# zkHubHQ/distributed-groth16

Measured on AMD Instinct MI355X. Metric: groth16_constraints_per_sec, higher is better.
Workload: dtype u32; 1 GPU; BN254 Groth16 prove from the matrices, synthetic R1CS with 2^20 - 2 constraints (3 nonzeros per row of A and B), 2^20 wires, 2 instance variables; r, s != 0 (R1CS x witness + 6 NTTs of 2^20 + 4 G1 MSMs + 1 G2 MSM); proving key RESIDENT as window tables (built once per key outside the timed region); curve=bn254, log_domain=20, parallelism=single GPU, key_table_bytes=6039807360, key_table_stride=1

## Files before the change

distributed-groth16_amd/csrc/msm_geom.h:

```cpp
#pragma once
#include <stddef.h>
#include <stdint.h>
#include <stdlib.h>

#ifndef DG_HD
#if defined(__HIPCC__)
#define DG_HD __host__ __device__ __forceinline__
#else
#define DG_HD inline
#endif
#endif

namespace dg16 {

constexpr unsigned kMinSegLog = 3, kMaxSegLog = 9;
constexpr unsigned kMinLanesLog = 18;
constexpr unsigned kGiantSegs = 64;
constexpr unsigned kGiantSlices = 64;
constexpr unsigned kGiantSliceSegs = 512;

struct MsmGeom {
  unsigned c;
  unsigned nwin;
  unsigned log_nb;
  unsigned seg_log;
  unsigned seg_cap;
  unsigned bw;
  unsigned table;
  unsigned rows;
  size_t region;
};

inline unsigned msm_window_bits(size_t n, bool table, unsigned scalar_bits = 0) {
  unsigned lg = 0;
  while (((size_t)1 << (lg + 1)) <= n) lg++;
  if (n > ((size_t)3 << lg) / 2) lg++;
  int c = table ? (int)lg - 3 : (int)lg - 4;
  if (table && c < 16) {
    c = (int)lg + 1 < 16 ? (int)lg + 1 : 16;
    if (scalar_bits && lg >= 13) {
      auto top = [&](int w) { const int bits = (int)scalar_bits + 1; return bits - ((bits + w - 1) / w - 1) * w; };
      const int t15 = top(15), t16 = top(16);
      if (t15 >= t16) c = (t15 > t16 || lg <= 16) ? 15 : 16;
    }
  }
  if (const char* e = getenv(table ? "DG16_MSM_TABLE_C" : "DG16_MSM_C")) c = atoi(e);
  int hi = table ? 20 : 16;
  if (c < 4) c = 4;
  if (c > hi) c = hi;
  return (unsigned)c;
}

inline MsmGeom msm_geometry(size_t n, unsigned scalar_bits, bool table = false, unsigned c_fixed = 0, unsigned stride = 1) {
  MsmGeom g;
  g.c = c_fixed ? c_fixed : msm_window_bits(n, table, table ? scalar_bits : 0);
  g.nwin = (scalar_bits + 1 + g.c - 1) / g.c;
  g.log_nb = g.c - 1;
  g.table = table ? 1u : 0u;
  if (stride < 1) stride = 1;
  if (stride > g.nwin) stride = g.nwin;
  g.bw = table ? stride : g.nwin;
  g.rows = (g.nwin + g.bw - 1) / g.bw;
  g.region = (size_t)g.rows * n;
  {
    size_t mean = g.region >> g.log_nb;
    unsigned lm = 0;
    while (((size_t)2 << lm) <= mean) lm++;
    unsigned le_all = 0;
    while (((size_t)2 << le_all) <= g.region * g.bw) le_all++;
    int sl = (int)le_all - 20;
    if (sl < 4) sl = 4;
    if (sl > 5) sl = 5;
    if (sl > (int)lm - 2) sl = (int)lm - 2;
    if (sl < 4) sl = 4;
    unsigned le = 0;
    while (((size_t)2 << le) <= (size_t)g.nwin * n) le++;
    int cap = (int)le - (int)kMinLanesLog;
    if (!table && le == 20 && cap < 4) cap = 4;
    if (sl > cap) sl = cap;
    g.seg_log = (unsigned)(sl < (int)kMinSegLog ? (int)kMinSegLog : sl > (int)kMaxSegLog ? (int)kMaxSegLog : sl);
    static const int seg_env = [] { const char* e = getenv("DG16_MSM_SEG_LOG"); return e ? atoi(e) : 0; }();
    if (seg_env >= (int)kMinSegLog && seg_env <= (int)kMaxSegLog) g.seg_log = (unsigned)seg_env;
  }
  g.seg_cap = (1u << g.log_nb) + (unsigned)((g.region + (1u << g.seg_log) - 1) >> g.seg_log);
  return g;
}

constexpr unsigned kScanBlock = 4096;

constexpr unsigned kPartScalars = 1024;
constexpr unsigned kPartMax = 256;
constexpr unsigned kPartMaxLowBits = 12;
constexpr unsigned kPartTileLog = 11;
constexpr unsigned kPartBlocks = 32;

struct PartGeom {
  unsigned low_bits, nparts, nblk1;
};
struct PartPlan {
  PartGeom pg;
  bool partitioned;
};
inline PartPlan msm_partition_plan(const MsmGeom& g, size_t n) {
  const size_t nbw = (size_t)g.bw << g.log_nb;
  unsigned lg_nbw = 0;
  while (((size_t)1 << lg_nbw) < nbw) lg_nbw++;
  static const int force_path = [] { const char* e = getenv("DG16_MSM_SORT"); return e ? atoi(e) : 0; }();
  PartPlan p;
  p.pg.low_bits = lg_nbw > 8 ? lg_nbw - 8 : 0;
  p.partitioned = p.pg.low_bits <= kPartMaxLowBits &&
                  (force_path == 2 || (force_path != 1 && (size_t)g.nwin * n >= ((size_t)1 << 18)));
  p.pg.nparts = (unsigned)((nbw + ((size_t)1 << p.pg.low_bits) - 1) >> p.pg.low_bits);
  p.pg.nblk1 = (unsigned)((n + kPartScalars - 1) / kPartScalars);
  return p;
}

constexpr unsigned kRowLog = 8;
struct RowGeom {
  unsigned row_log;
  unsigned rows_log;
};
inline RowGeom row_geometry(const MsmGeom& g) {
  RowGeom r;
  r.row_log = g.log_nb < kRowLog ? g.log_nb : kRowLog;
  r.rows_log = g.log_nb - r.row_log;
  return r;
}
constexpr size_t kLaneReduceMaxBuckets = 32768;

DG_HD void giant_geometry(unsigned nseg, unsigned& slices, unsigned& per) {
  slices = (nseg + kGiantSliceSegs - 1) / kGiantSliceSegs;
  if (slices > kGiantSlices) slices = kGiantSlices;
  per = (nseg + slices - 1) / slices;
  slices = (nseg + per - 1) / per;
}

constexpr int kGlvBits = 127;
constexpr int kGlv4Bits = 65;

struct PlainPlan {
  bool split;
  unsigned c_small;
  unsigned scalar_bits;
};
inline PlainPlan msm_plain_plan(bool nine_limbs, unsigned dim, size_t n, bool split_applies) {
  PlainPlan p{false, 0u, 0u};
  if (!split_applies || !n || !((size_t)dim * n * 40 < ((size_t)1 << 31))) return p;
  p.split = true;
  p.scalar_bits = dim == 2 ? (unsigned)kGlvBits : (unsigned)kGlv4Bits;
  if (dim == 2) {
    const unsigned c0 = msm_window_bits(2 * n, false);
    if (nine_limbs && (c0 == 7 || c0 == 9) && !getenv("DG16_MSM_C")) p.c_small = 8;
    if ((c0 == 14 || c0 == 15) && !getenv("DG16_MSM_C")) p.c_small = 16;
  }
  return p;
}

constexpr unsigned kMaxTableWin = 64;
inline unsigned table_stride_for(size_t full_bytes, size_t budget, unsigned nwin) {
  if (!budget || full_bytes <= budget || nwin <= 1) return 1;
  const size_t row = full_bytes / nwin;
  size_t rows_fit = budget / (row ? row : 1);
  if (rows_fit < 1) rows_fit = 1;
  unsigned k = (unsigned)((nwin + rows_fit - 1) / rows_fit);
  return k < 1 ? 1 : k > nwin ? nwin : k;
}

}
```

distributed-groth16_amd/csrc/msm_reduce_impl.h:

```cpp
#pragma once
#include "msm_impl.h"

#ifndef DG16_REDUCE_PRIO
#define DG16_REDUCE_PRIO 0
#endif
namespace dg16 {


template <class T>
__device__ __forceinline__ T lane_xor_words(const T& v, int mask) {
  static_assert(sizeof(T) % 4 == 0, "word-sized type");
  T r;
  const uint32_t* src = reinterpret_cast<const uint32_t*>(&v);
  uint32_t* dst = reinterpret_cast<uint32_t*>(&r);
#pragma unroll
  for (unsigned i = 0; i < sizeof(T) / 4; i++) dst[i] = (uint32_t)__shfl_xor((int)src[i], mask);
  return r;
}

template <class F>
__global__ void __launch_bounds__(256) msm_giant_kernel(MsmGeom g, unsigned wg_log, const unsigned* __restrict__ counts,
                                                         const unsigned* __restrict__ seg_off,
                                                         XYZZ29<F>* __restrict__ seg_sum,
                                                         const unsigned* __restrict__ giant_count,
                                                         const unsigned* __restrict__ giant_list, unsigned giant_cap) {
  __builtin_amdgcn_s_setprio(DG16_REDUCE_PRIO);
  __shared__ XYZZ29<F> sh[256];
  unsigned nwork = giant_count[1];
  if (nwork > 2 * giant_cap) nwork = 2 * giant_cap;
  const unsigned* work = giant_list + giant_cap;
  for (unsigned wi = blockIdx.x; wi < nwork; wi += gridDim.x) {
    const unsigned item = work[wi];
    const unsigned gid = giant_list[DG_IDX(11, item >> 6, giant_cap)], slice = item & 63;
    const unsigned wy = gid >> g.log_nb;
    const size_t gs = ((size_t)(wy % g.bw) << g.log_nb) + (gid & ((1u << g.log_nb) - 1));
    const unsigned k = (counts[gs] + (1u << g.seg_log) - 1) >> g.seg_log, first = seg_off[gs];
    const unsigned nseg = msm_nparts(first, k, wg_log);
    unsigned slices, per;
    giant_geometry(nseg, slices, per);
    XYZZ29<F>* sp = seg_sum + (size_t)wy * g.seg_cap;
    const unsigned lo = slice * per;
    const unsigned hi = lo + per < nseg ? lo + per : nseg;
    sh[threadIdx.x] = XYZZ29<F>::inf();
    __syncthreads();
    const unsigned iters = (hi - lo + 255) >> 8;
#pragma unroll 1
    for (unsigned step = 0; step < iters + 8; step++) {
      const XYZZ29<F>* b;
      bool on;
      if (step < iters) {
        const unsigned s = lo + step * 256 + threadIdx.x;
        on = s < hi;
        b = &sp[DG_IDX(12, msm_part_slot(first, on ? s : lo, wg_log), g.seg_cap)];
      } else {
        const unsigned stride = 128u >> (step - iters);
        on = threadIdx.x < stride;
        b = &sh[(threadIdx.x + stride) & 255];
      }
      if (on) XYZZ29<F>::add_mem(&sh[threadIdx.x], &sh[threadIdx.x], b);
      __syncthreads();
    }
    if (threadIdx.x == 0) sp[DG_IDX(12, msm_part_slot(first, lo, wg_log), g.seg_cap)] = sh[0];
    __syncthreads();
  }
}

template <class F>
__global__ void __launch_bounds__(64) msm_giant_fold_kernel(MsmGeom g, unsigned wg_log, const unsigned* __restrict__ counts,
                                                             const unsigned* __restrict__ seg_off,
                                                             const XYZZ29<F>* __restrict__ seg_sum,
                                                             XYZZ29<F>* __restrict__ buckets,
                                                             const unsigned* __restrict__ giant_count,
                                                             const unsigned* __restrict__ giant_list,
                                                             unsigned giant_cap) {
  __builtin_amdgcn_s_setprio(DG16_REDUCE_PRIO);
  __shared__ XYZZ29<F> sh[kGiantSlices];
  unsigned ng = *giant_count;
  if (ng > giant_cap) ng = giant_cap;
  for (unsigned gi = blockIdx.x; gi < ng; gi += gridDim.x) {
    const unsigned gid = giant_list[gi];
    const unsigned wy = gid >> g.log_nb;
    const size_t gs = ((size_t)(wy % g.bw) << g.log_nb) + (gid & ((1u << g.log_nb) - 1));
    const unsigned k = (counts[gs] + (1u << g.seg_log) - 1) >> g.seg_log, first = seg_off[gs];
    const unsigned nseg = msm_nparts(first, k, wg_log);
    unsigned slices, per;
    giant_geometry(nseg, slices, per);
    const XYZZ29<F>* sp = seg_sum + (size_t)wy * g.seg_cap;
    sh[threadIdx.x] = threadIdx.x < slices ? sp[DG_IDX(12, msm_part_slot(first, threadIdx.x * per, wg_log), g.seg_cap)] : XYZZ29<F>::inf();
    __syncthreads();
#pragma unroll 1
    for (unsigned stride = kGiantSlices / 2; stride > 0; stride >>= 1) {
      if (threadIdx.x < stride) XYZZ29<F>::add_mem(&sh[threadIdx.x], &sh[threadIdx.x], &sh[threadIdx.x + stride]);
      __syncthreads();
    }
    if (threadIdx.x == 0) buckets[gid] = sh[0];
    __syncthreads();
  }
}


constexpr unsigned kCoopTreeMax = 64;
template <class F>
__device__ __forceinline__ void tree_step_coop(XYZZ29<F>* sh, unsigned base, unsigned d) {
  const unsigned row16 = (threadIdx.x >> 4) & 15u;
#pragma unroll 1
  for (unsigned i = row16; i < d; i += 16) {
    const XYZZ29<F> v = add_wave29(sh[base + i], sh[base + i + d]);
    if ((threadIdx.x & 15u) == 0) sh[base + i] = v;
  }
}

template <class F>
__global__ void __launch_bounds__(256) msm_row_kernel(MsmGeom g, RowGeom rg, const XYZZ29<F>* __restrict__ buckets,
                                                       XYZZ29<F>* __restrict__ row_w, XYZZ29<F>* __restrict__ row_r) {
  __builtin_amdgcn_s_setprio(DG16_REDUCE_PRIO);
  __shared__ XYZZ29<F> sh[256];
  const unsigned c = threadIdx.x, row = 1u << rg.row_log;
  const size_t rid = ((size_t)blockIdx.y << rg.rows_log) + blockIdx.x;
  sh[c] = c < row ? buckets[(rid << rg.row_log) + c] : XYZZ29<F>::inf();
  __syncthreads();
#pragma unroll 1
  for (unsigned step = 0; step < 2 * rg.row_log; step++) {
    const bool scan = step < rg.row_log;
    const unsigned d = scan ? 1u << step : row >> (step - rg.row_log + 1);
    const bool on = scan ? c + d < row : c < d;
    if (step == rg.row_log && c == 0) row_r[rid] = sh[0];
    if (!scan && d <= kCoopTreeMax) {
      __syncthreads();
      tree_step_coop<F>(sh, 0u, d);
      __syncthreads();
      continue;
    }
    XYZZ29<F> v;
    if (on) XYZZ29<F>::add_mem(&v, &sh[c], &sh[(c + d) & 255]);
    __syncthreads();
    if (on) sh[c] = v;
    __syncthreads();
  }
  if (c == 0) {
    if (rg.row_log == 0) row_r[rid] = sh[0];
    row_w[rid] = sh[0];
  }
}

template <class F, int LANES>
__global__ void __launch_bounds__(LANES) msm_rowchunk_kernel(unsigned log_nb, unsigned k_log,
                                                              const XYZZ29<F>* __restrict__ buckets,
                                                              XYZZ29<F>* __restrict__ fold ) {
  __builtin_amdgcn_s_setprio(DG16_REDUCE_PRIO);
  constexpr unsigned LL = LANES == 256 ? 8u : 7u;
  static_assert(LANES == 256 || LANES == 128, "workgroup of 256 or 128 lanes");
  __shared__ XYZZ29<F> s_r[LANES];
  __shared__ XYZZ29<F> s_w[LANES];
  const unsigned j = threadIdx.x, K = 1u << k_log;
  const XYZZ29<F>* B = buckets + ((size_t)blockIdx.y << log_nb) + (((size_t)blockIdx.x * LANES + j) << k_log);
  XYZZ29<F>* out = fold + (size_t)blockIdx.y * 3 * 256;
  s_r[j] = XYZZ29<F>::inf();
  s_w[j] = XYZZ29<F>::inf();
  __syncthreads();
  const unsigned s_scan = 2 * K, s_tree = s_scan + LL, n_steps = s_tree + LL;
#pragma unroll 1
  for (unsigned step = 0; step < n_steps; step++) {
    const XYZZ29<F>*a, *b;
    XYZZ29<F>* dst;
    bool on = true;
    if (step < s_scan) {
      const bool even = (step & 1) == 0;
      dst = even ? &s_r[j] : &s_w[j];
      a = dst;
      b = even ? &B[K - 1 - (step >> 1)] : &s_r[j];
    } else if (step < s_tree) {
      const unsigned d = 1u << (step - s_scan);
      on = j + d < (unsigned)LANES;
      dst = &s_r[j];
      a = dst;
      b = &s_r[(j + d) & (LANES - 1)];
    } else {
      if (step == s_tree) {
        if (j == 0) {
          out[1 * 256 + blockIdx.x] = s_r[0];
          s_r[0] = XYZZ29<F>::inf();
        }
        __syncthreads();
      }
      const unsigned d = (unsigned)LANES >> (step - s_tree + 1);
      const unsigned c = j & (LANES / 2 - 1);
      XYZZ29<F>* arr = j < LANES / 2 ? s_r : s_w;
      on = c < d;
      dst = &arr[c];
      a = dst;
      b = &arr[(c + d) & (LANES - 1)];
    }
    XYZZ29<F> v;
    if (on) XYZZ29<F>::add_mem(&v, a, b);
    __syncthreads();
    if (on) *dst = v;
    __syncthreads();
  }
  if (j == 0) out[2 * 256 + blockIdx.x] = s_r[0];
  if (j == LANES / 2) out[0 * 256 + blockIdx.x] = s_w[0];
}

template <class F>
__global__ void __launch_bounds__(64) msm_rowfold_kernel(RowGeom rg, const XYZZ29<F>* __restrict__ row_w,
                                                          const XYZZ29<F>* __restrict__ row_r,
                                                          XYZZ29<F>* __restrict__ fold ) {
  __builtin_amdgcn_s_setprio(DG16_REDUCE_PRIO);
  __shared__ XYZZ29<F> st[64][2];
  const unsigned gid = blockIdx.x * 64 + threadIdx.x;
  const unsigned half = gid >> 8, t = gid & 255;
  const unsigned per_log = rg.rows_log - 8, per = 1u << per_log;
  const size_t base = ((size_t)blockIdx.y << rg.rows_log) + (size_t)t * per;
  XYZZ29<F>* run = &st[threadIdx.x][0];
  XYZZ29<F>* acc = &st[threadIdx.x][1];
  *run = XYZZ29<F>::inf();
  *acc = XYZZ29<F>::inf();
#pragma unroll 1
  for (unsigned k = 0; k < 2 * per; k++) {
    const unsigned j = per - 1 - (k >> 1);
    const bool first = (k & 1) == 0;
    const bool on = first ? (half == 1 && j + 1 < per) : true;
    const XYZZ29<F>* b = first ? run : (half == 0 ? row_w : row_r) + base + j;
    if (on) XYZZ29<F>::add_mem(first ? acc : run, first ? acc : run, b);
  }
  XYZZ29<F>* out = fold + (size_t)blockIdx.y * 3 * 256;
  out[half * 256 + t] = *run;
  if (half == 1) out[2 * 256 + t] = *acc;
}

struct TopGeom {
  unsigned folded, per_log, lanes, final_log, rows_log;
};
template <class F, int HALVES>
__global__ void __launch_bounds__(256 * HALVES) msm_top_kernel(TopGeom tg, const XYZZ29<F>* __restrict__ row_w,
                                                                const XYZZ29<F>* __restrict__ row_r,
                                                                const XYZZ29<F>* __restrict__ fold,
                                                                XYZZ29<F>* __restrict__ window_sums) {
  __builtin_amdgcn_s_setprio(DG16_REDUCE_PRIO);
  __shared__ XYZZ29<F> sh[256 * HALVES];
  __shared__ XYZZ29<F> keep;
  const unsigned t = threadIdx.x & 255;
  const bool folded = tg.folded != 0;
  const unsigned per_log = tg.per_log;
  const unsigned lanes = tg.lanes;
  const size_t base = (size_t)blockIdx.x << tg.rows_log;
  const XYZZ29<F>* fb = fold + (size_t)blockIdx.x * 3 * 256;
  XYZZ29<F>* me = &sh[threadIdx.x];
#pragma unroll 1
  for (int pass = 0; pass < 3 - HALVES; pass++) {
    const unsigned half = HALVES == 2 ? threadIdx.x >> 8 : (unsigned)pass;
    *me = t < lanes ? (folded ? fb[half * 256 + t] : (half == 0 ? row_w : row_r)[base + t]) : XYZZ29<F>::inf();
    __syncthreads();
    const unsigned s_tree = 9 + per_log, s_fin = s_tree + 8;
#pragma unroll 1
    for (unsigned step = 0; step < s_fin; step++) {
      XYZZ29<F> v;
      bool on = false, is_dbl = false;
      const XYZZ29<F>* b = me;
      if (step < 8) {
        const unsigned d = 1u << step;
        on = half == 1 && t + d < 256;
        b = me + (on ? d : 0);
      } else if (step < 8 + per_log) {
        on = half == 1;
        is_dbl = true;
      } else if (step == 8 + per_log) {
        on = half == 1 && folded && t < lanes;
        b = fb + 2 * 256 + (on ? t : 0);
      } else {
        const unsigned stride = 128u >> (step - s_tree);
        if (stride <= kCoopTreeMax) {
          tree_step_coop<F>(sh, (threadIdx.x >> 8) << 8, stride);
          __syncthreads();
          continue;
        }
        on = t < stride;
        b = me + (on ? stride : 0);
      }
      if (step == 8 && half == 1 && t == 0) *me = XYZZ29<F>::inf();
      if (on) {
        if (is_dbl) XYZZ29<F>::dbl_mem(&v, me);
        else XYZZ29<F>::add_mem(&v, me, b);
      }
      __syncthreads();
      if (on) *me = v;
      __syncthreads();
    }
    if (HALVES == 1 && pass == 0) {
      if (threadIdx.x == 0) keep = sh[0];
      __syncthreads();
    }
  }
  constexpr unsigned RES = HALVES == 2 ? 256u : 0u;
  if ((threadIdx.x >> 6) == (RES >> 6)) {
    if constexpr (lane29::enabled<F>()) {
      using FO = lane29::Ops<F>;
      typename FO::KT kc;
      kc.init();
      lane29::Pt<FO> a = lane29::load_pt<F>(kc, &sh[RES]);
#pragma unroll 1
      for (unsigned k = 0; k < tg.final_log; k++) a = lane29::dbl_pt<FO>(kc, a);
      a = lane29::add_pt<FO>(kc, a, lane29::load_pt<F>(kc, HALVES == 2 ? &sh[0] : &keep));
      lane29::store_pt<F>(kc, &window_sums[blockIdx.x], a);
    } else {
      XYZZ29<F> acc = sh[RES];
#pragma unroll 1
      for (unsigned k = 0; k < tg.final_log; k++) acc = dbl_wave29(acc);
      acc = add_wave29(acc, HALVES == 2 ? sh[0] : keep);
      if ((threadIdx.x & 63) == 0) window_sums[blockIdx.x] = acc;
    }
  }
}


constexpr size_t kLaneParallelMaxEntries = 4096;
template <class F>
constexpr int lane_reduce_radix_log() {
  return (FieldOf<F>::EXT || RR<typename FieldOf<F>::Params>::N > 9) ? 3 : 4;
}
template <class F, int RB>
__global__ void __launch_bounds__(64 << RB) msm_lane_reduce_kernel(const XYZZ29<F>* __restrict__ in,
                                                                    const XYZZ29<F>* __restrict__ in2, unsigned in_per_bw_log,
                                                                    unsigned g_log, unsigned u_log, int mode, unsigned k_log,
                                                                    XYZZ29<F>* __restrict__ out,
                                                                    XYZZ29<F>* __restrict__ window_sums) {
  const int level0 = mode == 0;
  if constexpr (lane29::enabled<F>()) {
    using FO = lane29::Ops<F>;
    using LPt = lane29::Pt<FO>;
    __shared__ XYZZ29<F> sA[2][1 << RB];
    __shared__ XYZZ29<F> sB[2][1 << RB];
    __builtin_amdgcn_s_setprio(DG16_REDUCE_PRIO);
    const unsigned w = threadIdx.x >> 6, G = 1u << g_log;
    typename FO::KT kc;
    kc.init();
    const size_t e = ((size_t)blockIdx.y << in_per_bw_log) + ((size_t)blockIdx.x << g_log) + w;
    LPt R, Y;
    if (mode == 0) {
      R = lane29::load_pt<F>(kc, &in[e]);
      Y = R;
    } else if (mode == 1) {
      Y = lane29::load_pt<F>(kc, &in[2 * e]);
      R = lane29::load_pt<F>(kc, &in[2 * e + 1]);
    } else if (mode == 2) {
      Y = lane29::load_pt<F>(kc, &in[e]);
      R = lane29::load_pt<F>(kc, &in2[e]);
    } else {
      const size_t t = ((size_t)blockIdx.x << g_log) + w;
      const XYZZ29<F>* f = in + (size_t)blockIdx.y * 3 * 256;
      LPt loc = lane29::load_pt<F>(kc, &f[2 * 256 + t]);
#pragma unroll 1
      for (unsigned k = 0; k < k_log; k++) loc = lane29::dbl_pt<FO>(kc, loc);
      Y = lane29::add_pt<FO>(kc, lane29::load_pt<F>(kc, &f[t]), loc);
      R = lane29::load_pt<F>(kc, &f[256 + t]);
    }
    unsigned buf = 0;
#pragma unroll 1
    for (unsigned d = 1; d < G; d <<= 1) {
      lane29::store_pt_raw<F>(kc, &sA[buf][w], R);
      __syncthreads();
      if (w + d < G) R = lane29::add_pt<FO>(kc, R, lane29::load_pt<F>(kc, &sA[buf][w + d]));
      buf ^= 1;
    }
    LPt X = R;
    if (w == 0) X = lane29::inf_pt<FO>(kc);
    bool first = true;
#pragma unroll 1
    for (unsigned d = G >> 1; d >= 1; d >>= 1) {
      lane29::store_pt_raw<F>(kc, &sA[buf][w], X);
      if (!level0) {
        if (first) lane29::store_pt_raw<F>(kc, &sB[buf][w], Y);
        else if (w >= 2 * d && w < 4 * d) lane29::store_pt_raw<F>(kc, &sB[buf][w - 2 * d], Y);
      }
      __syncthreads();
      if (w < d) X = lane29::add_pt<FO>(kc, X, lane29::load_pt<F>(kc, &sA[buf][w + d]));
      else if (!level0 && w < 2 * d)
        Y = lane29::add_pt<FO>(kc, lane29::load_pt<F>(kc, &sB[buf][w - d]), lane29::load_pt<F>(kc, &sB[buf][w]));
      buf ^= 1;
      first = false;
    }
    if (!level0 && G >= 2) {
      if (w == 1) lane29::store_pt_raw<F>(kc, &sB[buf][0], Y);
      __syncthreads();
      if (w == 0) Y = lane29::load_pt<F>(kc, &sB[buf][0]);
    }
    if (w != 0) return;
#pragma unroll 1
    for (unsigned k = 0; k < u_log; k++) X = lane29::dbl_pt<FO>(kc, X);
    const LPt Wp = lane29::add_pt<FO>(kc, level0 ? R : Y, X);
    if (window_sums) {
      lane29::store_pt<F>(kc, &window_sums[blockIdx.y], Wp);
    } else {
      const size_t o = ((size_t)blockIdx.y << (in_per_bw_log - g_log)) + blockIdx.x;
      lane29::store_pt_raw<F>(kc, &out[2 * o], Wp);
      lane29::store_pt_raw<F>(kc, &out[2 * o + 1], R);
    }
  }
}
template <class F>
__global__ void __launch_bounds__(64) msm_lane_reduce_serial_kernel(const XYZZ29<F>* __restrict__ in, unsigned in_per_bw_log,
                                                                     unsigned g_log, unsigned u_log, int level0,
                                                                     XYZZ29<F>* __restrict__ out,
                                                                     XYZZ29<F>* __restrict__ window_sums) {
  if constexpr (lane29::enabled<F>()) {
    using FO = lane29::Ops<F>;
    using LPt = lane29::Pt<FO>;
    const unsigned G = 1u << g_log;
    typename FO::KT kc;
    kc.init();
    const size_t e0 = ((size_t)blockIdx.y << in_per_bw_log) + ((size_t)blockIdx.x << g_log);
    const XYZZ29<F>* base = level0 ? in + e0 : in + 2 * e0;
    const unsigned stride = level0 ? 1u : 2u, roff = level0 ? 0u : 1u;
    LPt run = lane29::inf_pt<FO>(kc), acc = run, wsum = run;
    LPt rj = lane29::load_pt_words<F>(kc, base + (size_t)(G - 1) * stride + roff), wj = rj;
    if (!level0) wj = lane29::load_pt_words<F>(kc, base + (size_t)(G - 1) * stride);
#pragma unroll 1
    for (unsigned j = G - 1; j >= 1; j--) {
      const LPt rn = lane29::load_pt_words<F>(kc, base + (size_t)(j - 1) * stride + roff);
      LPt wn = rn;
      if (!level0) wn = lane29::load_pt_words<F>(kc, base + (size_t)(j - 1) * stride);
      run = lane29::add_pt<FO>(kc, run, lane29::with_inf_flag<FO>(rj));
      acc = lane29::add_pt<FO>(kc, acc, run);
      if (!level0) wsum = lane29::add_pt<FO>(kc, wsum, lane29::with_inf_flag<FO>(wj));
      rj = rn;
      wj = wn;
    }
    rj = lane29::with_inf_flag<FO>(rj);
    wj = lane29::with_inf_flag<FO>(wj);
    const LPt Rp = lane29::add_pt<FO>(kc, run, rj);
    if (!level0) wsum = lane29::add_pt<FO>(kc, wsum, wj);
#pragma unroll 1
    for (unsigned k = 0; k < u_log; k++) acc = lane29::dbl_pt<FO>(kc, acc);
    const LPt Wp = lane29::add_pt<FO>(kc, level0 ? Rp : wsum, acc);
    if (window_sums) {
      lane29::store_pt<F>(kc, &window_sums[blockIdx.y], Wp);
    } else {
      const size_t o = ((size_t)blockIdx.y << (in_per_bw_log - g_log)) + blockIdx.x;
      lane29::store_pt_raw<F>(kc, &out[2 * o], Wp);
      lane29::store_pt_raw<F>(kc, &out[2 * o + 1], Rp);
    }
  }
}
template <class F>
bool msm_lane_reduce(hipStream_t s, const MsmGeom& g, const MsmBuffers<F>& b) {
  if constexpr (!lane29::enabled<F>()) return false;
  else {
    const unsigned bwi = g.bw * b.ninst;
    if (!b.lane_tmp || !lane_reduce_applies<F>((size_t)bwi << g.log_nb)) return false;
    static const bool busy_off = [] { const char* e = getenv("DG16_NO_LANE_REDUCE_BUSY"); return e && atoi(e) != 0; }();
    if (b.busy_chip && busy_off) return false;
    constexpr int RB = lane_reduce_radix_log<F>();
    XYZZ29<F>* pong[2] = {b.lane_tmp, b.lane_tmp + (((size_t)bwi << g.log_nb) / 4 + 2)};
    const XYZZ29<F>* in = b.buckets;
    unsigned rem = g.log_nb, u_log = 0, per_log = g.log_nb, lvl = 0;
    do {
      const unsigned g_log = rem < (unsigned)RB ? rem : (unsigned)RB;
      const bool last = rem == g_log;
      XYZZ29<F>* out = pong[lvl & 1];
      const bool one_wave = b.busy_chip || ((size_t)bwi << per_log) > kLaneParallelMaxEntries;
      if (one_wave)
        hipLaunchKernelGGL((msm_lane_reduce_serial_kernel<F>), dim3(1u << (per_log - g_log), bwi), dim3(64), 0, s, in, per_log,
                           g_log, u_log, (int)(lvl == 0), out, last ? b.window_sums : (XYZZ29<F>*)nullptr);
      else
        hipLaunchKernelGGL((msm_lane_reduce_kernel<F, RB>), dim3(1u << (per_log - g_log), bwi), dim3(64u << g_log), 0, s, in,
                           (const XYZZ29<F>*)nullptr, per_log, g_log, u_log, lvl == 0 ? 0 : 1, 0u, out,
                           last ? b.window_sums : (XYZZ29<F>*)nullptr);
      in = out;
      rem -= g_log;
      per_log -= g_log;
      u_log += g_log;
      lvl++;
    } while (rem);
    return true;
  }
}

template <class F>
bool msm_lane_top(hipStream_t s, const MsmGeom& g, const MsmBuffers<F>& b, const TopGeom& tg) {
  if constexpr (!lane29::enabled<F>()) return false;
  else {
    const unsigned bwi = g.bw * b.ninst;
    static const bool off = [] { const char* e = getenv("DG16_NO_LANE_TOP"); return e && atoi(e) != 0; }();
    if (off || !b.top_tmp || b.busy_chip || (size_t)bwi * tg.lanes > kLaneParallelMaxEntries) return false;
    unsigned ll = 0;
    while ((1u << ll) < tg.lanes) ll++;
    if ((1u << ll) != tg.lanes) return false;
    constexpr int RB = lane_reduce_radix_log<F>();
    XYZZ29<F>* pong[2] = {b.top_tmp, b.top_tmp + (size_t)bwi * 64 + 4};
    const XYZZ29<F>* in = tg.folded ? b.fold : b.row_w;
    const XYZZ29<F>* in2 = tg.folded ? nullptr : b.row_r;
    unsigned rem = ll, per_log = ll, lvl = 0;
    unsigned u_log = tg.folded ? tg.final_log + tg.per_log : tg.final_log;
    do {
      const unsigned g_log = rem < (unsigned)RB ? rem : (unsigned)RB;
      const bool last = rem == g_log;
      XYZZ29<F>* out = pong[lvl & 1];
      hipLaunchKernelGGL((msm_lane_reduce_kernel<F, RB>), dim3(1u << (per_log - g_log), bwi), dim3(64u << g_log), 0, s, in, in2,
                         per_log, g_log, u_log, lvl ? 1 : (tg.folded ? 3 : 2), tg.final_log, out,
                         last ? b.window_sums : (XYZZ29<F>*)nullptr);
      in = out;
      in2 = nullptr;
      rem -= g_log;
      per_log -= g_log;
      u_log += g_log;
      lvl++;
    } while (rem);
    return true;
  }
}

inline void trace_point(hipStream_t s, const char* what) {
  static const bool on = [] { const char* e = getenv("DG16_TRACE"); return e && atoi(e) != 0; }();
  if (!on) return;
  static thread_local std::chrono::steady_clock::time_point last = std::chrono::steady_clock::now();
  hipError_t e = hipStreamSynchronize(s);
  auto now = std::chrono::steady_clock::now();
  fprintf(stderr, "[dg16 trace] %-24s %9.3f ms  %s\n", what, std::chrono::duration<double, std::milli>(now - last).count(),
          e == hipSuccess ? "" : hipGetErrorString(e));
  last = now;
}

template <class F>
void msm_bucket_phase(hipStream_t s, const MsmSort& st, const MsmBuffers<F>& b, bool out_affine, void* out_dev) {
  const MsmGeom& g = st.g;
  const unsigned bwi = g.bw * b.ninst;
  DG_BOUNDS_BIND();
  trace_point(s, "(before bucket phase)");
  if constexpr (FieldOf<F>::EXT) {
  } else {
    DG_HIP(hipMemsetAsync(b.giant, 0, 8, s));
    msm_finalize_phase<F>(s, st, b);
  }
  trace_point(s, "finalize");
  hipLaunchKernelGGL(msm_giant_kernel<F>, dim3(256), dim3(256), 0, s, g, msm_acc_wg_log<F>(), st.counts, st.seg_off,
                     b.seg_sum, b.giant, b.giant + 2, b.giant_cap);
  hipLaunchKernelGGL(msm_giant_fold_kernel<F>, dim3(64), dim3(64), 0, s, g, msm_acc_wg_log<F>(), st.counts, st.seg_off,
                     b.seg_sum, b.buckets, b.giant, b.giant + 2, b.giant_cap);
  trace_point(s, "giant + fold");
  if (msm_lane_reduce<F>(s, g, b)) {
    trace_point(s, "lane reduce");
    msm_tail_phase<F>(s, st, b, out_affine, out_dev);
    trace_point(s, "tail");
    DG_HIP(hipGetLastError());
    return;
  }
  constexpr int CH_LANES = sizeof(XYZZ29<F>) * 2 * 256 <= 150 * 1024 ? 256 : 128;
  constexpr unsigned CH_LL = CH_LANES == 256 ? 8u : 7u;
  unsigned k_log = 0;
  if (b.rg.row_log == kRowLog && g.log_nb >= CH_LL + 1) {
    const size_t total_rows = (size_t)bwi << b.rg.rows_log;
    while (k_log < 3 && (total_rows >> (k_log + 1)) >= 256 && g.log_nb >= CH_LL + k_log + 1) k_log++;
    if (total_rows < 1024) k_log = 0;
    if (total_rows < 1024 && RR<typename FieldOf<F>::Params>::N > 9 && g.table && g.region >= ((size_t)1 << 23)) {
      k_log = g.log_nb - CH_LL < 3 ? g.log_nb - CH_LL : 3;
    }
    if (k_log > 3) k_log = 3;
    if (k_log && g.log_nb - k_log - CH_LL > 8) k_log = 0;
  }
  TopGeom tg{};
  tg.rows_log = b.rg.rows_log;
  tg.final_log = b.rg.row_log;
  if (k_log) {
    const unsigned nsr_log = g.log_nb - k_log - CH_LL;
    DG_REQUIRE(nsr_log <= 8, DG16_ERR_UNSUPPORTED, "row chunks: more than 256 per bucket-window");
    hipLaunchKernelGGL((msm_rowchunk_kernel<F, CH_LANES>), dim3(1u << nsr_log, bwi), dim3(CH_LANES), 0, s, g.log_nb, k_log,
                       b.buckets, b.fold);
    trace_point(s, "row (chunks)");
    tg.folded = 1;
    tg.per_log = CH_LL;
    tg.lanes = 1u << nsr_log;
    tg.final_log = k_log;
  } else {
    hipLaunchKernelGGL(msm_row_kernel<F>, dim3(1u << b.rg.rows_log, bwi), dim3(256), 0, s, g, b.rg, b.buckets, b.row_w,
                       b.row_r);
    trace_point(s, "row");
    tg.folded = b.rg.rows_log > 8;
    tg.per_log = tg.folded ? b.rg.rows_log - 8 : 0;
    tg.lanes = tg.folded ? 256u : 1u << b.rg.rows_log;
    if (b.rg.rows_log > 8)
      hipLaunchKernelGGL(msm_rowfold_kernel<F>, dim3(8, bwi), dim3(64), 0, s, b.rg, b.row_w, b.row_r, b.fold);
  }
  constexpr int HALVES = sizeof(XYZZ29<F>) * 513 <= 160 * 1024 ? 2 : 1;
  if (!msm_lane_top<F>(s, g, b, tg))
    hipLaunchKernelGGL((msm_top_kernel<F, HALVES>), dim3(bwi), dim3(256 * HALVES), 0, s, tg, b.row_w, b.row_r,
                       b.fold, b.window_sums);
  trace_point(s, "top");
  msm_tail_phase<F>(s, st, b, out_affine, out_dev);
  trace_point(s, "tail");
  DG_HIP(hipGetLastError());
}

}
```

Before: 109.1 million constraints/s.

## Use wavefront shuffle reductions for giant buckets and add LDS-free light row chunks

The giant-bucket kernel now uses 64-lane workgroups that reduce segment sums in registers with cross-lane shuffles instead of a 256-entry shared-memory tree with barriers. A new light row-chunk kernel performs the bucket running-sum and lane scan with shuffles, and a row-form planner (overridable by environment variable) selects between the rows, chunks and light forms. This removes LDS traffic and barriers in the reduction, at the cost of fewer lanes per giant item and heavier register pressure. The light form is only chosen when forced through the environment.

```diff
diff --git a/distributed-groth16_amd/csrc/msm_geom.h b/distributed-groth16_amd/csrc/msm_geom.h
--- a/distributed-groth16_amd/csrc/msm_geom.h
+++ b/distributed-groth16_amd/csrc/msm_geom.h
@@ -128,6 +128,103 @@
 }
 constexpr size_t kLaneReduceMaxBuckets = 32768;
 
+enum RowForm : unsigned { kRowFormRows = 0, kRowFormChunks = 1, kRowFormLdsLight = 2 };
+constexpr unsigned kFoldEntries = 256;
+constexpr unsigned kFoldEntriesLog = 8;
+constexpr unsigned kLightLanesLog = 6;
+constexpr unsigned kLightChunkLog = 3;
+constexpr unsigned kLightMaxChunkLog = 5;
+static_assert((1u << (19 - kLightLanesLog - kLightMaxChunkLog)) <= kFoldEntries, "light chunks: a 2^19-bucket set fits fold");
+struct RowPlan {
+  unsigned form;
+  unsigned k_log;
+  unsigned lanes_log;
+  unsigned nsr_log;
+  bool over_lane_reduce;
+};
+inline int row_light_chunk_log(unsigned log_nb) {
+  if (log_nb < kLightLanesLog) return -1;
+  unsigned k = log_nb - kLightLanesLog < kLightChunkLog ? log_nb - kLightLanesLog : kLightChunkLog;
+  while (log_nb - kLightLanesLog - k > kFoldEntriesLog) k++;
+  return k <= kLightMaxChunkLog ? (int)k : -1;
+}
+enum LightKind : unsigned { kLightRun = 0, kLightAcc = 1, kLightScan = 2, kLightCross = 3, kLightTree = 4 };
+struct LightStep {
+  unsigned kind, idx, src;
+  bool on;
+};
+DG_HD unsigned light_steps(unsigned k_log) { return (2u << k_log) + 2 * kLightLanesLog; }
+DG_HD size_t light_first_bucket(unsigned sr, unsigned j, unsigned k_log) {
+  return (((size_t)sr << kLightLanesLog) + j) << k_log;
+}
+DG_HD LightStep light_step(unsigned step, unsigned k_log, unsigned j) {
+  const unsigned lanes = 1u << kLightLanesLog, s_scan = 2u << k_log, s_tree = s_scan + kLightLanesLog;
+  LightStep ls{kLightRun, 0u, j, true};
+  if (step < s_scan) {
+    ls.kind = (step & 1) ? kLightAcc : kLightRun;
+    ls.idx = (1u << k_log) - 1 - (step >> 1);
+  } else if (step < s_tree) {
+    const unsigned d = 1u << (step - s_scan);
+    ls.kind = kLightScan;
+    ls.on = j + d < lanes;
+    ls.src = (j + d) & (lanes - 1);
+  } else {
+    ls.kind = step == s_tree ? kLightCross : kLightTree;
+    ls.src = j ^ ((lanes / 2) >> (step - s_tree));
+  }
+  return ls;
+}
+
+inline int row_form_env() {
+  static const int v = [] {
+    const char* e = getenv("DG16_ROW_FORM");
+    if (!e) return -1;
+    const char* names[3] = {"rows", "chunks", "lds_light"};
+    for (int i = 0; i < 3; i++) {
+      const char *a = e, *b = names[i];
+      while (*a && *a == *b) a++, b++;
+      if (!*a && !*b) return i;
+    }
+    return -1;
+  }();
+  return v;
+}
+inline RowPlan row_form_plan(unsigned limbs, unsigned ext, bool busy_chip, bool table, size_t region, unsigned log_nb,
+                             unsigned bwi, bool lane_reduce, int forced = -1) {
+  RowPlan p{kRowFormRows, 0u, 0u, 0u, false};
+  const int kl = row_light_chunk_log(log_nb);
+  (void)busy_chip;
+  (void)lane_reduce;
+  const bool light = forced == (int)kRowFormLdsLight;
+  if (light && kl >= 0) {
+    p.form = kRowFormLdsLight;
+    p.k_log = (unsigned)kl;
+    p.lanes_log = kLightLanesLog;
+    p.nsr_log = log_nb - kLightLanesLog - p.k_log;
+    p.over_lane_reduce = forced == (int)kRowFormLdsLight;
+    return p;
+  }
+  if (forced == (int)kRowFormRows) return p;
+  const unsigned ll = (size_t)16 * limbs * ext * 2 * 256 <= 150 * 1024 ? 8u : 7u;
+  const unsigned row_log = log_nb < kRowLog ? log_nb : kRowLog, rows_log = log_nb - row_log;
+  unsigned k_log = 0;
+  if (row_log == kRowLog && log_nb >= ll + 1) {
+    const size_t total_rows = (size_t)bwi << rows_log;
+    while (k_log < 3 && (total_rows >> (k_log + 1)) >= 256 && log_nb >= ll + k_log + 1) k_log++;
+    if (total_rows < 1024) k_log = 0;
+    if ((forced == (int)kRowFormChunks) || (total_rows < 1024 && limbs > 9 && table && region >= ((size_t)1 << 23)))
+      k_log = log_nb - ll < 3 ? log_nb - ll : 3;
+    if (k_log && log_nb - k_log - ll > kFoldEntriesLog) k_log = 0;
+  }
+  if (k_log) {
+    p.form = kRowFormChunks;
+    p.k_log = k_log;
+    p.lanes_log = ll;
+    p.nsr_log = log_nb - k_log - ll;
+  }
+  return p;
+}
+
 DG_HD void giant_geometry(unsigned nseg, unsigned& slices, unsigned& per) {
   slices = (nseg + kGiantSliceSegs - 1) / kGiantSliceSegs;
   if (slices > kGiantSlices) slices = kGiantSlices;
diff --git a/distributed-groth16_amd/csrc/msm_reduce_impl.h b/distributed-groth16_amd/csrc/msm_reduce_impl.h
--- a/distributed-groth16_amd/csrc/msm_reduce_impl.h
+++ b/distributed-groth16_amd/csrc/msm_reduce_impl.h
@@ -18,14 +18,25 @@
   return r;
 }
 
-template <class F>
-__global__ void __launch_bounds__(256) msm_giant_kernel(MsmGeom g, unsigned wg_log, const unsigned* __restrict__ counts,
-                                                         const unsigned* __restrict__ seg_off,
-                                                         XYZZ29<F>* __restrict__ seg_sum,
-                                                         const unsigned* __restrict__ giant_count,
-                                                         const unsigned* __restrict__ giant_list, unsigned giant_cap) {
+template <class T>
+__device__ __forceinline__ T lane_from_words(const T& v, unsigned src) {
+  static_assert(sizeof(T) % 4 == 0, "word-sized type");
+  T r;
+  const uint32_t* in = reinterpret_cast<const uint32_t*>(&v);
+  uint32_t* dst = reinterpret_cast<uint32_t*>(&r);
+#pragma unroll
+  for (unsigned i = 0; i < sizeof(T) / 4; i++) dst[i] = (uint32_t)__shfl((int)in[i], (int)src);
+  return r;
+}
+
+template <class F>
+__global__ void __launch_bounds__(64) msm_giant_kernel(MsmGeom g, unsigned wg_log, const unsigned* __restrict__ counts,
+                                                        const unsigned* __restrict__ seg_off,
+                                                        XYZZ29<F>* __restrict__ seg_sum,
+                                                        const unsigned* __restrict__ giant_count,
+                                                        const unsigned* __restrict__ giant_list, unsigned giant_cap) {
   __builtin_amdgcn_s_setprio(DG16_REDUCE_PRIO);
-  __shared__ XYZZ29<F> sh[256];
+  constexpr unsigned LANES = 64, LL = 6;
   unsigned nwork = giant_count[1];
   if (nwork > 2 * giant_cap) nwork = 2 * giant_cap;
   const unsigned* work = giant_list + giant_cap;
@@ -41,27 +52,22 @@
     XYZZ29<F>* sp = seg_sum + (size_t)wy * g.seg_cap;
     const unsigned lo = slice * per;
     const unsigned hi = lo + per < nseg ? lo + per : nseg;
-    sh[threadIdx.x] = XYZZ29<F>::inf();
-    __syncthreads();
-    const unsigned iters = (hi - lo + 255) >> 8;
-#pragma unroll 1
-    for (unsigned step = 0; step < iters + 8; step++) {
-      const XYZZ29<F>* b;
-      bool on;
+    const unsigned iters = (hi - lo + LANES - 1) / LANES;
+    XYZZ29<F> run = XYZZ29<F>::inf();
+#pragma unroll 1
+    for (unsigned step = 0; step < iters + LL; step++) {
+      XYZZ29<F> b;
+      bool on = true;
       if (step < iters) {
-        const unsigned s = lo + step * 256 + threadIdx.x;
+        const unsigned s = lo + step * LANES + threadIdx.x;
         on = s < hi;
-        b = &sp[DG_IDX(12, msm_part_slot(first, on ? s : lo, wg_log), g.seg_cap)];
+        b = sp[DG_IDX(12, msm_part_slot(first, on ? s : lo, wg_log), g.seg_cap)];
       } else {
-        const unsigned stride = 128u >> (step - iters);
-        on = threadIdx.x < stride;
-        b = &sh[(threadIdx.x + stride) & 255];
+        b = lane_from_words(run, threadIdx.x ^ ((LANES / 2) >> (step - iters)));
       }
-      if (on) XYZZ29<F>::add_mem(&sh[threadIdx.x], &sh[threadIdx.x], b);
-      __syncthreads();
-    }
-    if (threadIdx.x == 0) sp[DG_IDX(12, msm_part_slot(first, lo, wg_log), g.seg_cap)] = sh[0];
-    __syncthreads();
+      if (on) XYZZ29<F>::add_mem(&run, &run, &b);
+    }
+    if (threadIdx.x == 0) sp[DG_IDX(12, msm_part_slot(first, lo, wg_log), g.seg_cap)] = run;
   }
 }
 
@@ -199,6 +205,46 @@
   }
   if (j == 0) out[2 * 256 + blockIdx.x] = s_r[0];
   if (j == LANES / 2) out[0 * 256 + blockIdx.x] = s_w[0];
+}
+
+template <class F>
+__global__ void __launch_bounds__(64) msm_rowchunk_light_kernel(unsigned log_nb, unsigned k_log,
+                                                                 const XYZZ29<F>* __restrict__ buckets,
+                                                                 XYZZ29<F>* __restrict__ fold ) {
+  __builtin_amdgcn_s_setprio(DG16_REDUCE_PRIO);
+  constexpr unsigned LANES = 1u << kLightLanesLog;
+  const unsigned j = threadIdx.x;
+  const XYZZ29<F>* B = buckets + ((size_t)blockIdx.y << log_nb) + light_first_bucket(blockIdx.x, j, k_log);
+  XYZZ29<F>* out = fold + (size_t)blockIdx.y * 3 * kFoldEntries;
+  XYZZ29<F> run = XYZZ29<F>::inf(), acc = XYZZ29<F>::inf();
+  const unsigned n_steps = light_steps(k_log);
+#pragma unroll 1
+  for (unsigned step = 0; step < n_steps; step++) {
+    const LightStep ls = light_step(step, k_log, j);
+    XYZZ29<F> a = run, b;
+    if (ls.kind == kLightRun) {
+      b = B[ls.idx];
+    } else if (ls.kind == kLightAcc) {
+      a = acc;
+      b = run;
+    } else {
+      XYZZ29<F> send = run;
+      if (ls.kind == kLightCross) {
+        if (j == 0) {
+          out[1 * kFoldEntries + blockIdx.x] = run;
+          run = XYZZ29<F>::inf();
+        }
+        send = j < LANES / 2 ? acc : run;
+        a = j < LANES / 2 ? run : acc;
+      }
+      b = lane_from_words(send, ls.src);
+    }
+    if (ls.on) XYZZ29<F>::add_mem(&a, &a, &b);
+    if (ls.kind == kLightAcc) acc = a;
+    else run = a;
+  }
+  if (j == 0) out[2 * kFoldEntries + blockIdx.x] = run;
+  if (j == LANES / 2) out[0 * kFoldEntries + blockIdx.x] = run;
 }
 
 template <class F>
@@ -532,12 +578,17 @@
     msm_finalize_phase<F>(s, st, b);
   }
   trace_point(s, "finalize");
-  hipLaunchKernelGGL(msm_giant_kernel<F>, dim3(256), dim3(256), 0, s, g, msm_acc_wg_log<F>(), st.counts, st.seg_off,
+  hipLaunchKernelGGL(msm_giant_kernel<F>, dim3(256), dim3(64), 0, s, g, msm_acc_wg_log<F>(), st.counts, st.seg_off,
                      b.seg_sum, b.giant, b.giant + 2, b.giant_cap);
   hipLaunchKernelGGL(msm_giant_fold_kernel<F>, dim3(64), dim3(64), 0, s, g, msm_acc_wg_log<F>(), st.counts, st.seg_off,
                      b.seg_sum, b.buckets, b.giant, b.giant + 2, b.giant_cap);
   trace_point(s, "giant + fold");
-  if (msm_lane_reduce<F>(s, g, b)) {
+  using FP = typename FieldOf<F>::Params;
+  constexpr unsigned EXT = FieldOf<F>::EXT ? 2u : 1u;
+  static_assert(sizeof(XYZZ29<F>) == (size_t)16 * RR<FP>::N * EXT, "row_form_plan's point size");
+  const RowPlan rp = row_form_plan((unsigned)RR<FP>::N, EXT, b.busy_chip, g.table != 0, g.region, g.log_nb, bwi,
+                                   b.lane_tmp && lane_reduce_applies<F>((size_t)bwi << g.log_nb), row_form_env());
+  if (!rp.over_lane_reduce && msm_lane_reduce<F>(s, g, b)) {
     trace_point(s, "lane reduce");
     msm_tail_phase<F>(s, st, b, out_affine, out_dev);
     trace_point(s, "tail");
@@ -545,30 +596,25 @@
     return;
   }
   constexpr int CH_LANES = sizeof(XYZZ29<F>) * 2 * 256 <= 150 * 1024 ? 256 : 128;
-  constexpr unsigned CH_LL = CH_LANES == 256 ? 8u : 7u;
-  unsigned k_log = 0;
-  if (b.rg.row_log == kRowLog && g.log_nb >= CH_LL + 1) {
-    const size_t total_rows = (size_t)bwi << b.rg.rows_log;
-    while (k_log < 3 && (total_rows >> (k_log + 1)) >= 256 && g.log_nb >= CH_LL + k_log + 1) k_log++;
-    if (total_rows < 1024) k_log = 0;
-    if (total_rows < 1024 && RR<typename FieldOf<F>::Params>::N > 9 && g.table && g.region >= ((size_t)1 << 23)) {
-      k_log = g.log_nb - CH_LL < 3 ? g.log_nb - CH_LL : 3;
-    }
-    if (k_log > 3) k_log = 3;
-    if (k_log && g.log_nb - k_log - CH_LL > 8) k_log = 0;
-  }
+  const unsigned k_log = rp.k_log;
   TopGeom tg{};
   tg.rows_log = b.rg.rows_log;
   tg.final_log = b.rg.row_log;
-  if (k_log) {
-    const unsigned nsr_log = g.log_nb - k_log - CH_LL;
-    DG_REQUIRE(nsr_log <= 8, DG16_ERR_UNSUPPORTED, "row chunks: more than 256 per bucket-window");
-    hipLaunchKernelGGL((msm_rowchunk_kernel<F, CH_LANES>), dim3(1u << nsr_log, bwi), dim3(CH_LANES), 0, s, g.log_nb, k_log,
-                       b.buckets, b.fold);
-    trace_point(s, "row (chunks)");
+  if (rp.form != kRowFormRows) {
+    DG_REQUIRE(rp.nsr_log <= kFoldEntriesLog, DG16_ERR_UNSUPPORTED, "row chunks: more than 256 per bucket-window");
+    if (rp.form == kRowFormLdsLight) {
+      hipLaunchKernelGGL(msm_rowchunk_light_kernel<F>, dim3(1u << rp.nsr_log, bwi), dim3(1u << kLightLanesLog), 0, s, g.log_nb,
+                         k_log, b.buckets, b.fold);
+      trace_point(s, "row (light chunks)");
+    } else {
+      DG_REQUIRE((1u << rp.lanes_log) == (unsigned)CH_LANES, DG16_ERR_UNSUPPORTED, "row chunks: workgroup size");
+      hipLaunchKernelGGL((msm_rowchunk_kernel<F, CH_LANES>), dim3(1u << rp.nsr_log, bwi), dim3(CH_LANES), 0, s, g.log_nb, k_log,
+                         b.buckets, b.fold);
+      trace_point(s, "row (chunks)");
+    }
     tg.folded = 1;
-    tg.per_log = CH_LL;
-    tg.lanes = 1u << nsr_log;
+    tg.per_log = rp.lanes_log;
+    tg.lanes = 1u << rp.nsr_log;
     tg.final_log = k_log;
   } else {
     hipLaunchKernelGGL(msm_row_kernel<F>, dim3(1u << b.rg.rows_log, bwi), dim3(256), 0, s, g, b.rg, b.buckets, b.row_w,
```

Result: no change. 108.5 million constraints/s (-0.6%).
